# memcached/memcached

Measured on AMD Instinct MI355X. Metric: CRC32C GiB/s over device-resident item batches; % of HBM roofline, higher is better.
Workload: dtype u8; 1 GPU; BASELINE configs[1]: 1 Mi items x 4096 B per GPU, stride 4096, one 32-lane group per item (K1 k_fixed<slice-by-4, 32 lanes, 8 x 16-B pieces per lane at 512-B spacing, non-temporal coalesced loads, half-item folds in the last-step tables, four items reduced per tree>); items_per_gpu=1048576, item_bytes=4096, parallelism=items sharded across 1 rank(s), no collective on the data path

## Files before the change

### memcached_amd/csrc/k_consts.h

```cpp
#pragma once

#include <stdint.h>

#if defined(__HIPCC__)
#define MCRC_HD __host__ __device__ __forceinline__
#else
#define MCRC_HD static inline
#endif

namespace mcrc_dev {

constexpr uint32_t kK1Bytes = 4096;
constexpr uint32_t kK1RoundSteps = 4;
static_assert(kK1RoundSteps >= 4 && kK1RoundSteps % 4 == 0, "a round is whole passes of K1's 4-step loop");
constexpr uint32_t kK1RoundsMinSteps = 32;
MCRC_HD uint64_t k1_rounds(uint64_t cg, uint32_t S) { return cg >= kK1RoundsMinSteps ? cg / S : 0; }
constexpr uint32_t kK1TailShift = 3;
constexpr uint32_t kK1TailSteps = 4;
constexpr uint32_t kK1TailPools = 16;
constexpr uint32_t kK1TailFloorSteps = 1u << kK1TailShift;
static_assert(kK1TailFloorSteps >= 8, "cg_s = 4 must leave a pool");
constexpr uint32_t kK1TailMinSteps = 40;
static_assert(kK1TailMinSteps >= kK1RoundsMinSteps && kK1TailMinSteps >= kK1TailFloorSteps, "");
struct K1Tail {
    uint64_t cg_s;
    uint64_t pool0;
    uint64_t nchunks;
};
MCRC_HD K1Tail k1_tail_split(uint64_t ngroups, uint64_t W) {
    const uint64_t cg = (ngroups + W - 1) / W;
    const uint64_t keep = (cg - (cg >> kK1TailShift)) & ~3ull;
    K1Tail t;
    t.cg_s = keep < 4 ? 4 : keep;
    t.pool0 = W * t.cg_s;
    t.nchunks = (ngroups - t.pool0 + kK1TailSteps - 1) / kK1TailSteps;
    return t;
}
MCRC_HD uint64_t k1_tail_pool_chunks(uint64_t nchunks, uint32_t t) {
    return nchunks > t ? (nchunks - t + kK1TailPools - 1) / kK1TailPools : 0;
}
struct K1Line {
    uint32_t v;
    uint32_t pad[63];
};
struct K1Ctl {
    K1Line head[kK1TailPools];
    K1Line done;
};
static_assert(sizeof(K1Line) == 256 && sizeof(K1Ctl) == 256 * (kK1TailPools + 1), "one line per counter");
constexpr uint32_t kRowBytes = 1024;
constexpr uint32_t kBlockBytes = 4 * kRowBytes;
constexpr uint32_t kSegBytes = 128 * 1024;
constexpr uint32_t kMaxSpan = 0x7fff0000u;
constexpr uint32_t kGridAlign = 128;
constexpr uint32_t kFragMax = 128;
constexpr uint32_t kWholeMax = 512;
MCRC_HD bool frag_drop(uint32_t len, uint64_t g1o, uint64_t vlen) {
    return len != 0 && (g1o <= kFragMax || vlen <= kWholeMax);
}
constexpr uint32_t kLineBytes = 128;
constexpr uint32_t kEpoch = 32;
MCRC_HD bool lines_fused(int64_t lines_bytes) {
    return lines_bytes >= (int64_t)(kBlockBytes - kLineBytes) && lines_bytes <= (int64_t)kBlockBytes;
}
constexpr uint32_t kSmallMax = 8192;
constexpr uint32_t kSpanBlock = 1024;
constexpr uint32_t kPlanThreads = 1024, kPlanPer = 2, kPlanTile = kPlanThreads * kPlanPer;
constexpr uint32_t kWalkWaves = 4;

}
```

### memcached_amd/csrc/k_fixed.h

```cpp
#pragma once

#include "k_common.h"

namespace mcrc_dev {

struct K1Half {
    uint4 d[4];
    uint32_t cin;
};
__device__ __forceinline__ uint32_t k1_half_value(const K1Half &r, const LaneCtx &c) {
    constexpr uint32_t kShift[3] = {kAuxShift0, kAuxShift1, kAuxShift2};
    uint32_t x[4];
#pragma unroll
    for (int k = 0; k < 4; ++k) x[k] = r.d[k].x;
#pragma unroll
    for (int i = 1; i < 4; ++i)
#pragma unroll
        for (int k = 0; k < 4; ++k) x[k] = step4_next(x[k], dw4(r.d[k], i), c);
#pragma unroll
    for (int k = 0; k < 4; ++k) x[k] = k < 3 ? step4_last_shifted(x[k], kShift[k]) : step4_next(x[k], 0u, c);
    return xor3(x[0], x[1], x[2]) ^ x[3];
}

__device__ __forceinline__ void k1_round_barrier() {
    __builtin_amdgcn_sched_barrier(0);
    __builtin_amdgcn_s_barrier();
    __builtin_amdgcn_sched_barrier(0);
}

struct K1NoProbe {
    __device__ __forceinline__ void steps(uint64_t ) const {}
    __device__ __forceinline__ void exit() const {}
};

template <bool CRCIN, bool NT, class Probe>
__device__ __forceinline__ void k_fixed_body(const uint8_t *__restrict__ base, uint64_t stride, uint64_t nitems,
                                             const uint4 *__restrict__ img, const uint32_t *__restrict__ crc_in,
                                             uint32_t *__restrict__ out, uint32_t nthreads, K1Ctl *__restrict__ ctl,
                                             const Probe &probe) {
    constexpr uint32_t IPW = 2;
    const uint32_t lane = threadIdx.x & 63u;
    const uint32_t li = lane & 31u;
    const uint32_t g = lane >> 5;
    const LaneCtx c = make_lane_ctx(li);
    const uint64_t waves = nthreads >> 6;
    const uint64_t gstep = gridDim.x * waves;
    const uint64_t ngroups = (nitems + IPW - 1) / IPW;
    uint64_t grp = __builtin_amdgcn_readfirstlane(blockIdx.x * (uint32_t)waves + (threadIdx.x >> 6));
    if (gstep % 65521u) grp = (grp * 65521u) % gstep;
    const bool tail = ctl != nullptr;
    const K1Tail tl = tail ? k1_tail_split(ngroups, gstep) : K1Tail{0, 0, 0};
    const uint64_t cg = tail ? tl.cg_s : (ngroups + gstep - 1) / gstep;
    uint64_t gend = min((grp + 1) * cg, ngroups);
    grp *= cg;
    uint64_t owed = k1_rounds(cg, kK1RoundSteps);
    const bool busy = grp < ngroups;
    uint64_t glast = gend - 1;
    auto item_of = [&](uint64_t gi) { return gi * IPW + g; };

    auto ldh = [&](K1Half &r, uint64_t gi, int q) {
        const bool real = gi < gend;
        const uint64_t gu = real ? gi : glast;
        const uint64_t first = gu * IPW;
        const uint8_t *wb = real ? base + first * stride : reinterpret_cast<const uint8_t *>(img);
        const uint32_t gl = first + g < nitems ? g : (uint32_t)(nitems - 1 - first);
        if (q == 0) {
            if constexpr (CRCIN) r.cin = crc_in[first + gl];
            else r.cin = 0u;
        }
        const uint32_t loff = (real ? gl * (uint32_t)stride : g * kK1Bytes) + li * kK1LaneBytes + 4u * kK1Piece * (uint32_t)q;
#pragma unroll
        for (int k = 0; k < 4; ++k)
            r.d[k] = NT ? ld16_nt(wb + loff + k * kK1Piece) : ld16((gbyte *)(wb + loff + k * kK1Piece));
        __builtin_amdgcn_sched_barrier(0);
    };
    auto half0 = [&](K1Half &m) {
        if (li == 0) m.d[0].x ^= ~m.cin;
        return apply_op<4>(kAuxSpanFold, k1_half_value(m, c));
    };
    auto part0 = [&](uint32_t u0, K1Half &m1) {
        return reduce_level<0>(u0 ^ k1_half_value(m1, c), (lane & 1u) == 0u);
    };
    K1Half h0, h1, h2, h3;
    auto step_even2 = [&](uint64_t a, uint64_t b) {
        ldh(h3, a, 1);
        const uint32_t u0 = half0(h0);
        ldh(h0, b, 0);
        return part0(u0, h1);
    };
    auto step_odd2 = [&](uint64_t a, uint64_t b) {
        ldh(h1, a, 1);
        const uint32_t u0 = half0(h2);
        ldh(h2, b, 0);
        return part0(u0, h3);
    };
    auto step_even = [&](uint64_t s) { return step_even2(s + 1, s + 2); };
    auto step_odd = [&](uint64_t s) { return step_odd2(s + 1, s + 2); };
    auto store4 = [&](uint32_t vab, uint32_t vc, uint32_t vd, uint64_t first) {
        const uint32_t raw = group_reduce32_quad_span(vab, group_pair_level1(vc, vd, lane), lane);
        const uint64_t item = item_of(first + (li & 3u));
        if (li < 4 && item < nitems) out[item] = ~raw;
    };
    uint64_t ran = 0;
    if (busy) {
        const uint64_t nsteps = gend - grp - (tail ? 4u : 0u);
        ldh(h0, grp, 0);
        ldh(h1, grp, 1);
        ldh(h2, grp + 1, 0);
        uint64_t k = 0;
        for (; k + 4 <= nsteps; k += 4) {
            const uint32_t va = step_even(grp);
            const uint32_t vb = step_odd(grp + 1);
            const uint32_t vab = group_pair_level1(va, vb, lane);
            const uint32_t vc = step_even(grp + 2);
            const uint32_t vd = step_odd(grp + 3);
            store4(vab, vc, vd, grp);
            grp += 4;
            if ((k + 4) % kK1RoundSteps == 0 && owed) {
                k1_round_barrier();
                --owed;
            }
            probe.steps(k + 4);
        }
        ran = k;
        for (; k + 2 <= nsteps; k += 2) {
            const uint32_t va = step_even(grp);
            const uint32_t vb = step_odd(grp + 1);
            const uint32_t raw = group_reduce32_pair_span(va, vb, lane);
            const uint64_t item = item_of(li == 0 ? grp : grp + 1);
            if (li < 2 && item < nitems) out[item] = ~raw;
            grp += 2;
        }
        if (nsteps & 1) {
            const uint32_t raw = group_reduce32_single_span(step_even(grp), lane);
            const uint64_t item = item_of(grp);
            if (li == 0 && item < nitems) out[item] = ~raw;
        }
    }
    for (; owed; --owed) k1_round_barrier();
    if (tail) {
        const uint32_t t = __builtin_amdgcn_readfirstlane(threadIdx.x >> 6);
        const uint64_t mine = k1_tail_pool_chunks(tl.nchunks, t);
        gend = ngroups;
        glast = ngroups - 1;
        typedef __attribute__((address_space(1))) uint32_t gu32;
        gu32 *head = (gu32 *)&ctl->head[t].v;
        asm volatile("" : "+v"(head));
        uint64_t cur = grp, nxt;
        do {
            uint32_t i = 0;
            if (lane == 0) i = __hip_atomic_fetch_add(head, 1u, __ATOMIC_RELAXED, __HIP_MEMORY_SCOPE_AGENT);
            const uint32_t va = step_even(cur);
            const uint32_t vb = step_odd(cur + 1);
            const uint32_t vab = group_pair_level1(va, vb, lane);
            i = __builtin_amdgcn_readfirstlane(i);
            nxt = i < mine ? tl.pool0 + ((uint64_t)i * kK1TailPools + t) * kK1TailSteps : ngroups;
            const uint32_t vc = step_even2(cur + 3, nxt);
            const uint32_t vd = step_odd2(nxt, nxt + 1);
            store4(vab, vc, vd, cur);
            cur = nxt;
            ran += 4;
            probe.steps(ran);
        } while (nxt < ngroups);
        k1_round_barrier();
        if (threadIdx.x < 64) {
            uint32_t old = 0;
            if (lane == 0) old = __hip_atomic_fetch_add(&ctl->done.v, 1u, __ATOMIC_RELAXED, __HIP_MEMORY_SCOPE_AGENT);
            if ((uint32_t)__builtin_amdgcn_readfirstlane(old) == gridDim.x - 1 && lane <= kK1TailPools)
                __hip_atomic_store(lane < kK1TailPools ? &ctl->head[lane].v : &ctl->done.v, 0u, __ATOMIC_RELAXED,
                                   __HIP_MEMORY_SCOPE_AGENT);
        }
    }
    probe.exit();
}

template <bool CRCIN, bool NT>
__global__ __launch_bounds__(1024) void k_fixed(const uint8_t *__restrict__ base, uint64_t stride,
                                                uint64_t nitems, const uint4 *__restrict__ img,
                                                const uint32_t *__restrict__ crc_in,
                                                uint32_t *__restrict__ out, K1Ctl *__restrict__ ctl) {
    extern __shared__ __attribute__((aligned(16))) char smem[];
    load_tables(smem, img, kLdsImageK1Bytes);
    k_fixed_body<CRCIN, NT>(base, stride, nitems, img, crc_in, out, blockDim.x, ctl, K1NoProbe{});
}

}
```

Measured before the change: 6416 GiB/s.

## Interleave K1 wave work within a workgroup window instead of contiguous per-wave ranges

Replaces the scrambled contiguous per-wave range assignment with a window order. In the default window-pass mode, the waves of one workgroup take consecutive 4-step passes of a shared block-sized window, so concurrently running waves read neighbouring memory. This is meant to improve DRAM page and channel locality and to reduce scattered access from the old modular scramble. It adds index arithmetic and a remainder segment per wave, and the tail and non-4-multiple paths become more complex.

```diff
diff --git a/memcached_amd/csrc/k_consts.h b/memcached_amd/csrc/k_consts.h
--- a/memcached_amd/csrc/k_consts.h
+++ b/memcached_amd/csrc/k_consts.h
@@ -15,6 +15,44 @@
 static_assert(kK1RoundSteps >= 4 && kK1RoundSteps % 4 == 0, "a round is whole passes of K1's 4-step loop");
 constexpr uint32_t kK1RoundsMinSteps = 32;
 MCRC_HD uint64_t k1_rounds(uint64_t cg, uint32_t S) { return cg >= kK1RoundsMinSteps ? cg / S : 0; }
+enum K1Order : uint32_t { kK1OrderRanges = 0, kK1OrderWindowStep = 1, kK1OrderWindowPass = 2 };
+MCRC_HD uint64_t k1_scramble(uint64_t i, uint64_t n) { return n % 65521u ? (i * 65521u) % n : i; }
+MCRC_HD K1Order k1_order_for(K1Order o, uint64_t cg) { return cg >= kK1RoundsMinSteps ? o : kK1OrderRanges; }
+struct K1Walk {
+    uint64_t first, sstep, pstep, rfirst, end;
+};
+MCRC_HD K1Walk k1_walk(K1Order o, bool scramble, uint32_t b, uint32_t t, uint32_t nwg, uint32_t wv, uint64_t cg) {
+    const uint64_t whole = cg & ~3ull, rem = cg & 3u;
+    K1Walk k;
+    if (o == kK1OrderRanges) {
+        k.first = k1_scramble(b * wv + t, (uint64_t)nwg * wv) * cg;
+        k.sstep = 1, k.pstep = 4;
+        k.rfirst = k.first + whole;
+        k.end = k.first + cg;
+        return k;
+    }
+    const uint64_t base = (scramble ? k1_scramble(b, nwg) : b) * wv * cg;
+    k.pstep = 4ull * wv;
+    if (o == kK1OrderWindowPass) {
+        k.first = base + 4ull * t;
+        k.sstep = 1;
+        k.rfirst = base + wv * whole + rem * t;
+        k.end = k.rfirst + rem;
+    } else {
+        k.first = base + t;
+        k.sstep = wv;
+        k.rfirst = base + wv * whole + t;
+        k.end = base + wv * cg;
+    }
+    return k;
+}
+MCRC_HD uint64_t k1_group(K1Order o, bool scramble, uint32_t b, uint32_t t, uint64_t q, uint32_t j, uint32_t nwg,
+                          uint32_t wv, uint64_t cg) {
+    const K1Walk k = k1_walk(o, scramble, b, t, nwg, wv, cg);
+    return (q < cg / 4 ? k.first + q * k.pstep : k.rfirst) + j * k.sstep;
+}
+constexpr K1Order kK1Order = kK1OrderWindowPass;
+constexpr bool kK1WindowScramble = false;
 constexpr uint32_t kK1TailShift = 3;
 constexpr uint32_t kK1TailSteps = 4;
 constexpr uint32_t kK1TailPools = 16;
diff --git a/memcached_amd/csrc/k_fixed.h b/memcached_amd/csrc/k_fixed.h
--- a/memcached_amd/csrc/k_fixed.h
+++ b/memcached_amd/csrc/k_fixed.h
@@ -33,7 +33,7 @@
     __device__ __forceinline__ void exit() const {}
 };
 
-template <bool CRCIN, bool NT, class Probe>
+template <bool CRCIN, bool NT, class Probe, K1Order ORD = kK1Order, bool SCR = kK1WindowScramble>
 __device__ __forceinline__ void k_fixed_body(const uint8_t *__restrict__ base, uint64_t stride, uint64_t nitems,
                                              const uint4 *__restrict__ img, const uint32_t *__restrict__ crc_in,
                                              uint32_t *__restrict__ out, uint32_t nthreads, K1Ctl *__restrict__ ctl,
@@ -46,13 +46,16 @@
     const uint64_t waves = nthreads >> 6;
     const uint64_t gstep = gridDim.x * waves;
     const uint64_t ngroups = (nitems + IPW - 1) / IPW;
-    uint64_t grp = __builtin_amdgcn_readfirstlane(blockIdx.x * (uint32_t)waves + (threadIdx.x >> 6));
-    if (gstep % 65521u) grp = (grp * 65521u) % gstep;
     const bool tail = ctl != nullptr;
     const K1Tail tl = tail ? k1_tail_split(ngroups, gstep) : K1Tail{0, 0, 0};
     const uint64_t cg = tail ? tl.cg_s : (ngroups + gstep - 1) / gstep;
-    uint64_t gend = min((grp + 1) * cg, ngroups);
-    grp *= cg;
+    const uint32_t wslot = __builtin_amdgcn_readfirstlane(threadIdx.x >> 6);
+    const K1Order ord = k1_order_for(ORD, cg);
+    const K1Walk wk = k1_walk(ord, SCR, blockIdx.x, wslot, gridDim.x, (uint32_t)waves, cg);
+    uint64_t grp = wk.first;
+    const uint64_t ss = ORD == kK1OrderWindowStep ? wk.sstep : 1;
+    const uint64_t ps = ORD == kK1OrderRanges ? 4 : wk.pstep;
+    uint64_t gend = min(wk.end, ngroups);
     uint64_t owed = k1_rounds(cg, kK1RoundSteps);
     const bool busy = grp < ngroups;
     uint64_t glast = gend - 1;
@@ -94,28 +97,28 @@
         ldh(h2, b, 0);
         return part0(u0, h3);
     };
-    auto step_even = [&](uint64_t s) { return step_even2(s + 1, s + 2); };
-    auto step_odd = [&](uint64_t s) { return step_odd2(s + 1, s + 2); };
-    auto store4 = [&](uint32_t vab, uint32_t vc, uint32_t vd, uint64_t first) {
+    auto store4 = [&](uint32_t vab, uint32_t vc, uint32_t vd, uint64_t first, uint64_t sp) {
         const uint32_t raw = group_reduce32_quad_span(vab, group_pair_level1(vc, vd, lane), lane);
-        const uint64_t item = item_of(first + (li & 3u));
+        const uint64_t item = item_of(first + (li & 3u) * (uint32_t)sp);
         if (li < 4 && item < nitems) out[item] = ~raw;
     };
     uint64_t ran = 0;
     if (busy) {
-        const uint64_t nsteps = gend - grp - (tail ? 4u : 0u);
+        const uint64_t nsteps = (ord != kK1OrderRanges ? cg : gend - grp) - (tail ? 4u : 0u);
+        const uint64_t nwhole = (nsteps + (tail ? 4u : 0u)) & ~3ull;
         ldh(h0, grp, 0);
         ldh(h1, grp, 1);
-        ldh(h2, grp + 1, 0);
+        ldh(h2, grp + ss, 0);
         uint64_t k = 0;
         for (; k + 4 <= nsteps; k += 4) {
-            const uint32_t va = step_even(grp);
-            const uint32_t vb = step_odd(grp + 1);
+            const uint64_t nxt = ord == kK1OrderRanges || k + 8 <= nwhole ? grp + ps : wk.rfirst;
+            const uint32_t va = step_even2(grp + ss, grp + 2 * ss);
+            const uint32_t vb = step_odd2(grp + 2 * ss, grp + 3 * ss);
             const uint32_t vab = group_pair_level1(va, vb, lane);
-            const uint32_t vc = step_even(grp + 2);
-            const uint32_t vd = step_odd(grp + 3);
-            store4(vab, vc, vd, grp);
-            grp += 4;
+            const uint32_t vc = step_even2(grp + 3 * ss, nxt);
+            const uint32_t vd = step_odd2(nxt, nxt + ss);
+            store4(vab, vc, vd, grp, ss);
+            grp = nxt;
             if ((k + 4) % kK1RoundSteps == 0 && owed) {
                 k1_round_barrier();
                 --owed;
@@ -124,41 +127,42 @@
         }
         ran = k;
         for (; k + 2 <= nsteps; k += 2) {
-            const uint32_t va = step_even(grp);
-            const uint32_t vb = step_odd(grp + 1);
+            const uint32_t va = step_even2(grp + ss, grp + 2 * ss);
+            const uint32_t vb = step_odd2(grp + 2 * ss, grp + 3 * ss);
             const uint32_t raw = group_reduce32_pair_span(va, vb, lane);
-            const uint64_t item = item_of(li == 0 ? grp : grp + 1);
+            const uint64_t item = item_of(li == 0 ? grp : grp + ss);
             if (li < 2 && item < nitems) out[item] = ~raw;
-            grp += 2;
+            grp += 2 * ss;
         }
         if (nsteps & 1) {
-            const uint32_t raw = group_reduce32_single_span(step_even(grp), lane);
+            const uint32_t raw = group_reduce32_single_span(step_even2(grp + ss, grp + 2 * ss), lane);
             const uint64_t item = item_of(grp);
             if (li == 0 && item < nitems) out[item] = ~raw;
         }
     }
     for (; owed; --owed) k1_round_barrier();
     if (tail) {
-        const uint32_t t = __builtin_amdgcn_readfirstlane(threadIdx.x >> 6);
+        const uint32_t t = wslot;
         const uint64_t mine = k1_tail_pool_chunks(tl.nchunks, t);
         gend = ngroups;
         glast = ngroups - 1;
         typedef __attribute__((address_space(1))) uint32_t gu32;
         gu32 *head = (gu32 *)&ctl->head[t].v;
         asm volatile("" : "+v"(head));
-        uint64_t cur = grp, nxt;
+        uint64_t cur = grp, nxt, sp = ss;
         do {
             uint32_t i = 0;
             if (lane == 0) i = __hip_atomic_fetch_add(head, 1u, __ATOMIC_RELAXED, __HIP_MEMORY_SCOPE_AGENT);
-            const uint32_t va = step_even(cur);
-            const uint32_t vb = step_odd(cur + 1);
+            const uint32_t va = step_even2(cur + sp, cur + 2 * sp);
+            const uint32_t vb = step_odd2(cur + 2 * sp, cur + 3 * sp);
             const uint32_t vab = group_pair_level1(va, vb, lane);
             i = __builtin_amdgcn_readfirstlane(i);
             nxt = i < mine ? tl.pool0 + ((uint64_t)i * kK1TailPools + t) * kK1TailSteps : ngroups;
-            const uint32_t vc = step_even2(cur + 3, nxt);
+            const uint32_t vc = step_even2(cur + 3 * sp, nxt);
             const uint32_t vd = step_odd2(nxt, nxt + 1);
-            store4(vab, vc, vd, cur);
+            store4(vab, vc, vd, cur, sp);
             cur = nxt;
+            if constexpr (ORD == kK1OrderWindowStep) sp = 1;
             ran += 4;
             probe.steps(ran);
         } while (nxt < ngroups);
```

Result: faster. 6570 GiB/s, median of 6 (+2.4%).
